# kscalelabs/kbot-joystick

Hardware: AMD Instinct MI355X
Metric: env-steps/sec (whole node), K-Bot joystick 8192 envs @1/2/4/8 MI355X (higher is better)
Workload: dtype f32; 1 GPU; kbot-headless, 8192 envs/GPU, flat ground, fixed joystick command (0.5,0,0), full iteration: 100-step rollout + PPO update (batch 512/GPU, 3 passes, LSTM hidden 256, depth 2); envs_per_gpu=8192, rollout_steps=100, batch_size_per_gpu=512, num_passes=3, hidden_size=256, deterministic_update=True, parallelism=env-sharded dp1, grad all-reduce per optimizer step

## Files before the change

kbot-joystick_amd/csrc/kbj_nn.hip:

```cpp
#include <hip/hip_runtime.h>
#include <vector>
#include <cmath>
#include <cstdlib>
#include <algorithm>
#include <type_traits>
#include "kbj_ctx.h"
#include "kbj_gemm.h"
#include "kbj_nn_kernels.h"
#include "kbj_lstm_seq.h"
#include "kbj_lstm_bwd16.h"
#include "kbj_deploy.h"
#include "kbj_terminal_value.h"

using namespace kbj;

namespace {

constexpr int MAXD = KBJ_MAX_DEPTH;

struct NetOff {
  size_t w_in, b_in, w_ih[MAXD], w_hh[MAXD], b[MAXD], w_out, b_out;
  int nin, nout, ld_obs;
};

// ... 443 lines not shown

int ev_record(kbj_ctx* ctx, hipEvent_t ev, hipStream_t on) { KBJ_HIP(ctx, hipEventRecord(ev, on)); return 0; }
int ev_wait(kbj_ctx* ctx, hipStream_t st, hipEvent_t ev) { KBJ_HIP(ctx, hipStreamWaitEvent(st, ev, 0)); return 0; }
int hop(kbj_ctx* ctx, hipStream_t from, hipStream_t to, hipEvent_t ev) { return ev_record(ctx, ev, from) || ev_wait(ctx, to, ev) ? -1 : 0; }

void pad_params(kbj_ctx* ctx, hipStream_t s, const float* user, float* internal) {
  NnWs& w = *ws_of(ctx);
  hipLaunchKernelGGL(pad_params_kernel, g1(w.nparams), dim3(256), 0, s, w.pad_desc, w.npad, const_cast<float*>(user), internal, w.nparams, 0);
}
void unpad_params(kbj_ctx* ctx, hipStream_t s, const float* internal, float* user) {
  NnWs& w = *ws_of(ctx);
  hipLaunchKernelGGL(pad_params_kernel, g1(w.nparams), dim3(256), 0, s, w.pad_desc, w.npad, user, const_cast<float*>(internal), w.nparams, 1);
}
void repitch_hc(kbj_ctx* ctx, hipStream_t s, const float* src, float* dst, int ws, int wd) {
  NnWs& w = *ws_of(ctx);
  const size_t rows = (size_t)2 * w.D * w.N;
  repitch_pad_launch(s, src, dst, rows, ws, wd);
}
kbj_carry pad_carry(kbj_ctx* ctx, hipStream_t s, const kbj_carry& c) {
  NnWs& w = *ws_of(ctx);
  kbj_carry p = c;
  for (int k = 0; k < 4; ++k)
    if (carry_hc(c, k) && w.phc[k]) { repitch_hc(ctx, s, carry_hc(c, k), w.phc[k], w.Hu, w.H); carry_hc(p, k) = w.phc[k]; }
  return p;
}
void unpad_carry(kbj_ctx* ctx, hipStream_t s, const kbj_carry& c) {
  NnWs& w = *ws_of(ctx);
  for (int k = 0; k < 4; ++k)
    if (carry_hc(c, k) && w.phc[k]) repitch_hc(ctx, s, w.phc[k], carry_hc(c, k), w.H, w.Hu);
}
kbj_traj pad_traj_carry0(kbj_ctx* ctx, hipStream_t s, const kbj_traj& tr) {
  NnWs& w = *ws_of(ctx);
  kbj_traj p = tr;
  for (int k = 0; k < 4; ++k)
    if (traj_carry0(tr, k) && w.pc0[k]) { repitch_hc(ctx, s, traj_carry0(tr, k), w.pc0[k], w.Hu, w.H); traj_carry0(p, k) = w.pc0[k]; }
  return p;
}


enum HeadKind {
  HEAD_SAMPLE,
  HEAD_VALUE,
  HEAD_LPF,
  HEAD_NONE
};
struct RolloutNet { hipStream_t lane; int type; bool step_kernel, folded0, mirrored, terminal; int tile; HeadKind head; float *hc, *lpf, *X, *G, *Out, *obs_m, **rH; };
struct RolloutPlan { RolloutNet net[4]; int nnets; bool serial; hipStream_t side; float* term_rows; hipEvent_t ev_term; };

RolloutPlan rollout_plan(kbj_ctx* ctx, const kbj_carry& carry, bool serial) {
  NnWs& w = *ws_of(ctx); const Sched& sc = w.sched;
  RolloutPlan p{};
  p.nnets = w.nnets; p.serial = serial;
  p.side = serial ? ctx->stream : ctx->side[0];
  p.term_rows = ctx->cfg_h.gae_terminal_value ? w.term_rows : nullptr;
  p.ev_term = p.term_rows && !serial ? ctx->ev_term : nullptr;
  const HeadKind heads[4] = {HEAD_SAMPLE, HEAD_VALUE, HEAD_LPF, HEAD_NONE};
  float* const lpf[4] = {carry.lpf_d, nullptr, carry.lpf_mirror_d, nullptr};
  for (int n = 0; n < p.nnets; ++n) {
    RolloutNet& q = p.net[n]; q.type = n & 1;
    q.lane = n == 0 ? ctx->stream : p.side;
    q.step_kernel = sc.rollout_step && n == 0;
    q.tile = sc.rollout_step && n > 0 ? 0 : -1;
    q.folded0 = q.step_kernel && sc.fold_actor && w.net[0].ld_obs == KBJ_LD_ACTOR;
    q.head = heads[n]; q.mirrored = n >= 2;
    q.terminal = n == 1 && p.term_rows != nullptr;
    q.hc = carry_hc(carry, n); q.lpf = lpf[n];
    q.X = w.rX[n]; q.G = w.rG[n]; q.Out = w.rOut[n]; q.obs_m = q.mirrored ? w.rObsM[q.type] : nullptr; q.rH = w.rH[n];
  }
  return p;
}

struct StepRows {
  const float *actor_obs, *critic_obs; float *aux, *action, *logp, *value, *actor_next, *critic_next, *aux_next, *qstate;
  uint32_t step_index; int argmax, parity;
  float* value_term;
};

void terminal_value_launch(hipStream_t st, const float* par, const NetOff& o, int N, int width, int D, const float* hc, const float* rows, const float* done_d, int done_stride,
                           float* value) {
  TermValueArgs a{};
  a.params = par; a.rows = rows; a.hc = hc; a.done = done_d; a.done_stride = done_stride; a.value = value;
  a.N = N; a.H = width; a.D = D; a.nin = o.nin; a.ld = o.ld_obs;
  a.w_in = o.w_in; a.b_in = o.b_in; a.w_out = o.w_out; a.b_out = o.b_out;
  for (int l = 0; l < D; ++l) { a.w_ih[l] = o.w_ih[l]; a.w_hh[l] = o.w_hh[l]; a.b[l] = o.b[l]; }
  critic_terminal_value_launch(st, a);
}

struct Rollout {
  kbj_ctx* ctx; const float* params; const RolloutPlan p; uint32_t seed;
  NnWs& w = *ws_of(ctx); const kbj_config& c = ctx->cfg_h; const int N = w.N, H = w.H;
  const HeadParams hp{c.min_std, c.max_std, c.var_scale, c.lpf_alpha, w.net[0].ld_obs};

  float* c_plane(const RolloutNet& q, int l) { return q.hc + (size_t)(2 * l + 1) * N * H; }
  float* h_plane(const RolloutNet& q, int l, bool partner) { return partner ? q.rH[l] : q.hc + (size_t)(2 * l) * N * H; }

  void fold_actor_weights(hipStream_t s) {
    if (!p.net[0].folded0) return;
    const NetOff& oa = w.net[0];
    GemmArgs g{params + oa.w_ih[0], params + oa.w_in, w.Weff, nullptr, 4 * H, oa.nin, H, H, oa.nin, oa.ld_obs, 0, 1, nullptr};
    gemm_launch<true, false>(s, g);
    matvec_launch(s, params + oa.w_ih[0], params + oa.b_in, params + oa.b[0], 4 * H, H, w.beff);
  }

  void repitch_input_weights(hipStream_t s, int k_lo = 0, int k_hi = 2) {
    for (int k = k_lo; k < k_hi; ++k) {
      const NetOff& o = w.net[k];
      if (o.nin != o.ld_obs) repitch_rows_launch(s, params + o.w_in, H, o.nin, o.ld_obs, w.WinP[k]);
    }
  }

  const float* observation_rows(const RolloutNet& q, const StepRows& v) {
    const float* obs = q.type == 0 ? v.actor_obs : v.critic_obs;
    if (!q.mirrored) return obs;
    mirror_rows_launch(q.lane, obs, q.obs_m, (size_t)N, w.net[q.type].ld_obs, w.mtab[q.type]);
    return q.obs_m;
  }

  void input_projection(const RolloutNet& q, const float* obs) {
    const NetOff& o = w.net[q.type];
    if (o.nin != o.ld_obs) linear_fwd(q.lane, obs, o.ld_obs, w.WinP[q.type], o.ld_obs, params + o.b_in, q.X, H, N, H, o.ld_obs, 0);
    else linear_fwd(q.lane, obs, o.ld_obs, params + o.w_in, o.nin, params + o.b_in, q.X, H, N, H, o.nin, 0);
  }

  const float* layers_step_kernel(const RolloutNet& q, const float* obs, int parity) {
    const NetOff& o = w.net[q.type];
    const float* x = q.X;
    for (int l = 0; l < w.D; ++l) {
      float* h_out = h_plane(q, l, parity == 0);
      StepArgs sa{x, H, 0, params + o.w_ih[l], H, params + o.w_hh[l], params + o.b[l], h_plane(q, l, parity != 0), h_out, c_plane(q, l), N};
      if (l == 0 && q.folded0) { sa.X = obs; sa.ldx = o.ld_obs; sa.kx = o.nin; sa.Wih = w.Weff; sa.ldw = o.ld_obs; sa.bias = w.beff; }
      if (lstm_step(ctx, q.lane, H, sa)) return nullptr;
      x = h_out;
    }
    return x;
  }

  const float* layers_gemm_cell(const RolloutNet& q) {
    const NetOff& o = w.net[q.type];
    const float* x = q.X;
    for (int l = 0; l < w.D; ++l) {
      float *h = h_plane(q, l, false), *cc = c_plane(q, l);
      GemmArgs g{x, params + o.w_ih[l], q.G, params + o.b[l], N, 4 * H, 2 * H, H, H, 4 * H, 0, 1, nullptr};
      g.A2 = h; g.B2 = params + o.w_hh[l]; g.k1 = H;
      g.x3 = w.sched.gemm_x3 ? 1 : 0;
      gemm_launch<true, true>(q.lane, g, q.tile);
      CellFwdArgs2 ca;
      ca.a[0] = CellFwdArgs{q.G, cc, h, cc, nullptr, nullptr, nullptr, nullptr, N, H};
      lstm_cell_fwd_launch(q.lane, ca, 1);
      x = h;
    }
    return x;
  }

  void head(const RolloutNet& q, const float* x, const float* obs, const StepRows& v) {
    const NetOff& o = w.net[q.type];
    if (q.head == HEAD_SAMPLE)
      actor_head_fused_launch(q.lane, x, H, params + o.w_out, params + o.b_out, obs, q.lpf, w.joint_bias_d, hp, seed, (uint32_t)c.env_id_offset, v.step_index, v.argmax, N,
                              v.action, v.logp);
    else if (q.head == HEAD_VALUE) critic_value_fused_launch(q.lane, x, H, params + o.w_out, params + o.b_out, N, v.value);
    else if (q.head == HEAD_LPF) {
      linear_fwd(q.lane, x, H, params + o.w_out, H, params + o.b_out, q.Out, 40, N, o.nout, H, 0);
      actor_head_lpf_launch(q.lane, q.Out, obs, q.lpf, w.joint_bias_d, c.lpf_alpha, N, w.net[0].ld_obs);
    }
  }

  int net_step(const RolloutNet& q, const StepRows& v) {
    const float* obs = observation_rows(q, v);
    if (!q.folded0) input_projection(q, obs);
    const float* x = q.step_kernel ? layers_step_kernel(q, obs, v.parity) : layers_gemm_cell(q);
    if (!x) return -1;
    head(q, x, obs, v);
    return 0;
  }

  void carry_reset(const RolloutNet& q, const float* done_d, int done_stride, int parity) {
    CarryPlanes cp;
    cp.n = 2 * w.D;
    for (int l = 0; l < w.D; ++l) { cp.p[2 * l] = h_plane(q, l, q.step_kernel && parity != 0); cp.p[2 * l + 1] = c_plane(q, l); }
    carry_reset_launch(q.lane, cp, N, H, q.lpf, done_d, done_stride);
  }

  int terminal_value(const RolloutNet& q, const StepRows& v) {
    if (!q.terminal) return 0;
    terminal_value_launch(q.lane, params, w.net[q.type], N, H, w.D, q.hc, p.term_rows, v.aux + KBJ_AUX_DONE, KBJ_AUX_SIZE, v.value_term);
    return p.ev_term ? ev_record(ctx, p.ev_term, q.lane) : 0;
  }
  int terminal_rows_free(hipStream_t s, bool first_step) { return p.ev_term && !first_step ? ev_wait(ctx, s, p.ev_term) : 0; }

  int planes_home() {
    for (int n = 0; n < p.nnets; ++n)
      for (int l = 0; l < w.D && p.net[n].step_kernel; ++l)
        KBJ_HIP(ctx, hipMemcpyAsync(h_plane(p.net[n], l, false), h_plane(p.net[n], l, true), (size_t)N * H * sizeof(float), hipMemcpyDeviceToDevice, ctx->stream));
    return 0;
  }

  int critic_tail(const float* critic_obs_d, const float* critic_hc_d, int hc_width, float* value_d) {
    RolloutNet q = p.net[1];
    q.hc = w.tail_hc;
    if (hc_width == H) KBJ_HIP(ctx, hipMemcpyAsync(w.tail_hc, critic_hc_d, (size_t)2 * w.D * N * H * sizeof(float), hipMemcpyDeviceToDevice, q.lane));
    else repitch_hc(ctx, q.lane, critic_hc_d, w.tail_hc, hc_width, H);
    StepRows v{};
    v.critic_obs = critic_obs_d; v.value = value_d;
    return net_step(q, v);
  }
};

int policy_step_body(kbj_ctx* ctx, const float* params_d, const float* actor_obs_d, const float* critic_obs_d, kbj_carry* carry, uint32_t seed,
                     uint32_t step_index, int argmax, float* action_d, float* logp_d, float* value_d) {
  kbj_nn_drop_prefetch(ctx);
  KbjTimed timed(ctx, true);
  Rollout r{ctx, params_d, rollout_plan(ctx, *carry, true), seed};
  r.repitch_input_weights(ctx->stream);
  r.fold_actor_weights(ctx->stream);
  const StepRows v{actor_obs_d, critic_obs_d, nullptr, action_d, logp_d, value_d, nullptr, nullptr, nullptr, nullptr, step_index, argmax, 0};
  for (int n = 0; n < r.p.nnets; ++n) if (r.net_step(r.p.net[n], v)) return -1;
  if (r.planes_home()) return -1;
  KBJ_CHECK_LAUNCH(ctx, "kbj_policy_step");
  return 0;
}

int rollout_body(kbj_ctx* ctx, const float* params_d, kbj_carry* carry, uint32_t seed, uint32_t first_step_index, kbj_traj* tr) {
  NnWs& w = *ws_of(ctx);
  const size_t N = w.N, T = tr->T, la = w.net[0].ld_obs, lc = w.net[1].ld_obs, lx = KBJ_AUX_SIZE;
  hipStream_t s = ctx->stream;
  kbj_nn_drop_prefetch(ctx);
  const struct { float* a; size_t ld; } rows[3] = {{tr->actor_obs_d, la}, {tr->critic_obs_d, lc}, {tr->aux_d, lx}};
  for (const auto& r : rows) KBJ_HIP(ctx, hipMemcpyAsync(r.a, r.a + T * N * r.ld, N * r.ld * sizeof(float), hipMemcpyDeviceToDevice, s));
  for (int n = 0; n < w.nnets; n += 2) {
    for (int k = n; k < n + 2; ++k)
      KBJ_HIP(ctx, hipMemcpyAsync(traj_carry0(*tr, k), carry_hc(*carry, k), 2 * w.D * N * w.H * sizeof(float), hipMemcpyDeviceToDevice, s));
    KBJ_HIP(ctx, hipMemcpyAsync(n ? tr->carry0_lpf_mirror_d : tr->carry0_lpf_d, n ? carry->lpf_mirror_d : carry->lpf_d, N * KBJ_NU * sizeof(float), hipMemcpyDeviceToDevice, s));
  }
  const char* pipe_env = getenv("KBJ_ROLLOUT_PIPELINE");
  Rollout r{ctx, params_d, rollout_plan(ctx, *carry, pipe_env && atoi(pipe_env) == 0), seed};
  const RolloutPlan& p = r.p;
  r.fold_actor_weights(s);
  r.repitch_input_weights(s);
  if (!p.serial && hop(ctx, s, p.side, ctx->ev_fork)) return -1;
  for (size_t t = 0; t < T; ++t) {
    const StepRows v{tr->actor_obs_d + t * N * la, tr->critic_obs_d + t * N * lc, tr->aux_d + t * N * lx, tr->action_d + t * N * KBJ_NU, tr->logp_d + t * N, tr->value_d + t * N,
                     tr->actor_obs_d + (t + 1) * N * la, tr->critic_obs_d + (t + 1) * N * lc, tr->aux_d + (t + 1) * N * lx,
                     tr->qstate_d ? tr->qstate_d + t * N * KBJ_QSTATE_SIZE : nullptr, first_step_index + (uint32_t)t, ctx->rollout_argmax, (int)(t & 1),
                     p.term_rows ? w.value_term + t * N : nullptr};
    const float* done = v.aux + KBJ_AUX_DONE;
    for (int n = 0; n < p.nnets; ++n) if (r.net_step(p.net[n], v)) return -1;
    if (r.terminal_rows_free(s, t == 0)) return -1;
    const int rc = kbj_env_step_all(ctx, s, v.action, v.aux, v.actor_next, v.critic_next, v.aux_next, v.qstate, p.term_rows);
    if (rc) return rc;
    r.carry_reset(p.net[0], done, KBJ_AUX_SIZE, (v.parity + 1) & 1);
    if (!p.serial && hop(ctx, s, p.side, ctx->ev_side[0])) return -1;
    for (int n = 1; n < p.nnets; ++n) {
      if (r.terminal_value(p.net[n], v)) return -1;
      r.carry_reset(p.net[n], done, KBJ_AUX_SIZE, (v.parity + 1) & 1);
    }
  }
  if (ctx->cfg_h.gae_tail_value && tr->value_tail_d && r.critic_tail(tr->critic_obs_d + T * N * lc, carry->critic_hc_d, w.H, tr->value_tail_d)) return -1;
  KBJ_CHECK_LAUNCH(ctx, "kbj_rollout");
  if (!p.serial && hop(ctx, p.side, s, ctx->ev_side[0])) return -1;
  if ((T & 1) && r.planes_home()) return -1;
  return kbj_rewards(ctx, tr->aux_d, (int)T, tr->reward_d, tr->reward_comps_d);
}

}

extern "C" {

int kbj_mirror_table(const void* model_blob, size_t model_bytes, int critic, int32_t* src_h, float* mul_h, float* add_h) {
  if (!model_blob || !src_h || !mul_h || !add_h || model_bytes != sizeof(kbj_model)) return kbj_fail(nullptr, "kbj_mirror_table: bad argument");
  std::vector<MirrorEntry> ta, tc;
  build_mirror_tables(*reinterpret_cast<const kbj_model*>(model_blob), ta, tc);
  const std::vector<MirrorEntry>& t = critic ? tc : ta;
  for (size_t k = 0; k < t.size(); ++k) { src_h[k] = t[k].src; mul_h[k] = t[k].mul; add_h[k] = t[k].add; }
  return (int)t.size();
}

size_t kbj_param_count(const kbj_config* cfg) { return layout_params(*cfg, cfg->hidden_size).nparams; }
size_t kbj_actor_param_count(const kbj_config* cfg) { return layout_params(*cfg, cfg->hidden_size).nactor; }

int kbj_init_params(kbj_ctx* ctx, uint32_t seed, float* params_d) {
  if (!ctx || !params_d) return kbj_fail(ctx, "kbj_init_params: null argument");
  KBJ_HIP(ctx, hipSetDevice(ctx->device));
  NnWs& w = *ws_of(ctx);
  const ParamLayout& u = w.user;
  int H = w.Hu;
  uint32_t leaf = 0;
  auto fill = [&](size_t off, size_t n, int fan_in) {
    init_uniform_launch(ctx->stream, params_d + off, n, 1.0f / std::sqrt((float)fan_in), seed, leaf++);
  };
  for (int n = 0; n < 2; ++n) {
    const NetOff& o = u.net[n];
    fill(o.w_in, (size_t)H * o.nin, o.nin); fill(o.b_in, H, o.nin);
    for (int l = 0; l < w.D; ++l) { fill(o.w_ih[l], (size_t)4 * H * H, H); fill(o.w_hh[l], (size_t)4 * H * H, H); fill(o.b[l], (size_t)4 * H, H); }
    fill(o.w_out, (size_t)o.nout * H, H); fill(o.b_out, o.nout, H);
  }
  KBJ_CHECK_LAUNCH(ctx, "init_uniform_kernel");
  return 0;
}

int kbj_policy_step(kbj_ctx* ctx, const float* params_d, const float* actor_obs_d, const float* critic_obs_d, kbj_carry* carry, uint32_t seed,
                    uint32_t step_index, int argmax, float* action_d, float* logp_d, float* value_d) {
  if (!ctx || !params_d || !actor_obs_d || !critic_obs_d || !carry || !action_d || !logp_d || !value_d) return kbj_fail(ctx, "kbj_policy_step: null argument");
  KBJ_HIP(ctx, hipSetDevice(ctx->device));
  NnWs& w = *ws_of(ctx);
  if (mirror_arrays_missing(w.mirror, carry, nullptr)) return kbj_fail(ctx, "kbj_policy_step: the mirror losses are enabled, the carry needs the mirror-branch arrays");
  if (!w.padded()) return policy_step_body(ctx, params_d, actor_obs_d, critic_obs_d, carry, seed, step_index, argmax, action_d, logp_d, value_d);
  pad_params(ctx, ctx->stream, params_d, w.pparams);
  kbj_carry pc = pad_carry(ctx, ctx->stream, *carry);
  const int rc = policy_step_body(ctx, w.pparams, actor_obs_d, critic_obs_d, &pc, seed, step_index, argmax, action_d, logp_d, value_d);
  unpad_carry(ctx, ctx->stream, *carry);
  return rc;
}

int kbj_carry_reset(kbj_ctx* ctx, kbj_carry* carry, const float* done_d, int done_stride) {
  if (!ctx || !carry || !done_d) return kbj_fail(ctx, "kbj_carry_reset: null argument");
  KBJ_HIP(ctx, hipSetDevice(ctx->device));
  NnWs& w = *ws_of(ctx);
  if (mirror_arrays_missing(w.mirror, carry, nullptr)) return kbj_fail(ctx, "kbj_carry_reset: the mirror losses are enabled, the carry needs the mirror-branch arrays");
  const kbj_carry pc = w.padded() ? pad_carry(ctx, ctx->stream, *carry) : *carry;
  Rollout r{ctx, nullptr, rollout_plan(ctx, pc, true), 0};
  for (int n = 0; n < r.p.nnets; ++n) r.carry_reset(r.p.net[n], done_d, done_stride, 0);
  if (w.padded()) unpad_carry(ctx, ctx->stream, *carry);
  KBJ_CHECK_LAUNCH(ctx, "carry_reset_kernel");
  return 0;
}

// ... 563 lines not shown
```

kbot-joystick_amd/csrc/kbj_nn_kernels.h:

```cpp
#pragma once
#include <hip/hip_runtime.h>
#include <stdint.h>
#include <cmath>
#include <vector>
#include "kbj_model.h"
#include "kbj_lstm_seq.h"

namespace kbj {

constexpr float kLog2Pi = 1.8378770664093453f;
inline dim3 g1(size_t n, int bs = 256) { return dim3((unsigned)((n + bs - 1) / bs)); }

__device__ __forceinline__ float sigmoidf_(float x) { return __builtin_amdgcn_rcpf(1.0f + __expf(-x)); }
__device__ __forceinline__ float tanhf_(float x) { float xc = fminf(fmaxf(x, -15.0f), 15.0f); return 1.0f - 2.0f * __builtin_amdgcn_rcpf(1.0f + __expf(2.0f * xc)); }
__device__ __forceinline__ float softplusf_(float x) { return x > 20.0f ? x : log1pf(expf(x)); }

__device__ __forceinline__ void lstm_cell_point(float pi, float pf, float pg, float po, float c_prev, float& i, float& f, float& gg, float& o, float& c, float& tc) {
  i = sigmoidf_(pi); f = sigmoidf_(pf); gg = tanhf_(pg); o = sigmoidf_(po);
  c = f * c_prev + i * gg;
  tc = tanhf_(c);
}
struct CellFwdArgs {
  float* G; const float* c_prev; float* h_out; float* c_out; float* hm_next; float* cm_next; float* tanhc; const float* keep;
  int M, H;
};
struct CellFwdArgs2 { CellFwdArgs a[2]; };
__global__ void lstm_cell_fwd_kernel(CellFwdArgs2 args) {
  const CellFwdArgs& a = args.a[blockIdx.y];
  int idx = blockIdx.x * blockDim.x + threadIdx.x;
  if (idx >= a.M * a.H) return;
  int m = idx / a.H, u = idx - m * a.H;
  float* g = a.G + (size_t)m * 4 * a.H;
  float i, f, gg, o, c, tc;
  lstm_cell_point(g[u], g[a.H + u], g[2 * a.H + u], g[3 * a.H + u], a.c_prev[idx], i, f, gg, o, c, tc);
  float h = o * tc;
  g[u] = i; g[a.H + u] = f; g[2 * a.H + u] = gg; g[3 * a.H + u] = o;
  a.h_out[idx] = h;
  a.c_out[idx] = c;
  if (a.hm_next) { float k = a.keep[m]; a.hm_next[idx] = h * k; a.cm_next[idx] = c * k; a.tanhc[idx] = tc; }
}
inline void lstm_cell_fwd_launch(hipStream_t st, const CellFwdArgs2& a, int count) {
  hipLaunchKernelGGL(lstm_cell_fwd_kernel, dim3((a.a[0].M * a.a[0].H + 255) / 256, count), dim3(256), 0, st, a);
}

__device__ __forceinline__ uint32_t nn_rotl32(uint32_t x, int r) { return (x << r) | (x >> (32 - r)); }
__device__ __forceinline__ void nn_threefry(uint32_t k0, uint32_t k1, uint32_t c0, uint32_t c1, uint32_t& o0, uint32_t& o1) {
  const int rot[8] = {13, 15, 26, 6, 17, 29, 16, 24};
  uint32_t ks[3] = {k0, k1, k0 ^ k1 ^ 0x1BD11BDAu};
  uint32_t x0 = c0 + ks[0], x1 = c1 + ks[1];
#pragma unroll
  for (int g = 0; g < 5; ++g) {
#pragma unroll
    for (int r = 0; r < 4; ++r) { x0 += x1; x1 = nn_rotl32(x1, rot[(g & 1) * 4 + r]); x1 ^= x0; }
    x0 += ks[(g + 1) % 3]; x1 += ks[(g + 2) % 3] + (uint32_t)(g + 1);
  }
  o0 = x0; o1 = x1;
}

struct HeadParams { float min_std, max_std, var_scale, alpha; int ld_obs; };
constexpr int HEAD_ENVS = 16;
constexpr int HEAD_WAVES = 4;
typedef float head_f32x4 __attribute__((ext_vector_type(4)));
__global__ __launch_bounds__(64 * HEAD_WAVES) void actor_head_fused_kernel(const float* __restrict__ hin , int H, const float* __restrict__ Wout ,
                                                                          const float* __restrict__ bout, const float* __restrict__ obs ,
                                                                          float* __restrict__ lpf, const float* __restrict__ joint_bias, HeadParams hp, uint32_t seed,
                                                                          uint32_t env_off, uint32_t step, int argmax, int N, float* __restrict__ action,
                                                                          float* __restrict__ logp) {
  __shared__ float outs[HEAD_WAVES][HEAD_ENVS][49];
  __shared__ float lps[HEAD_WAVES][HEAD_ENVS][KBJ_NU + 1];
  const int lane = threadIdx.x & 63, wv = threadIdx.x >> 6, g = lane >> 4, c = lane & 15;
  const int n0 = (blockIdx.x * HEAD_WAVES + wv) * HEAD_ENVS;
  if (n0 < N) {
    const float* arow = hin + (size_t)min(n0 + c, N - 1) * H + 4 * g;
    const float* brow[3] = {Wout + (size_t)c * H + 4 * g, Wout + (size_t)(16 + c) * H + 4 * g, Wout + (size_t)min(32 + c, 2 * KBJ_NU - 1) * H + 4 * g};
    head_f32x4 acc[3] = {{0, 0, 0, 0}, {0, 0, 0, 0}, {0, 0, 0, 0}};
    for (int k = 0; k < H; k += 16) {
      const head_f32x4 a = *reinterpret_cast<const head_f32x4*>(arow + k);
#pragma unroll
      for (int t = 0; t < 3; ++t) {
        const head_f32x4 b = *reinterpret_cast<const head_f32x4*>(brow[t] + k);
#pragma unroll
        for (int q = 0; q < 4; ++q) acc[t] = __builtin_amdgcn_mfma_f32_16x16x4f32(a[q], b[q], acc[t], 0, 0, 0);
      }
    }
#pragma unroll
    for (int t = 0; t < 3; ++t)
#pragma unroll
      for (int r = 0; r < 4; ++r) outs[wv][4 * g + r][16 * t + c] = acc[t][r];
  }
  __syncthreads();
  if (n0 < N) {
    for (int item = lane; item < HEAD_ENVS * KBJ_NU; item += 64) {
      const int e = item / KBJ_NU, j = item - e * KBJ_NU, n = n0 + e;
      float lp = 0;
      if (n < N) {
        const float om = outs[wv][e][j] + bout[j], os = outs[wv][e][KBJ_NU + j] + bout[KBJ_NU + j];
        float mean = om + joint_bias[j] + (j >= 10 ? obs[(size_t)n * hp.ld_obs + KBJ_OBS_CMD + 6 + (j - 10)] : 0.0f);
        float sd = fminf((softplusf_(os) + hp.min_std) * hp.var_scale, hp.max_std);
        float y0 = lpf[n * KBJ_NU + j];
        float y = y0 + hp.alpha * (mean - y0);
        lpf[n * KBJ_NU + j] = y;
        float a = y;
        if (!argmax) {
          uint32_t b0, b1;
          nn_threefry(seed ^ ((uint32_t)KBJ_RNG_ACTION * 0x9E3779B9u), env_off + (uint32_t)n, step, (uint32_t)j, b0, b1);
          float u1 = (float)((b0 >> 8) + 1u) * (1.0f / 16777216.0f), u2 = (float)(b1 >> 8) * (1.0f / 16777216.0f);
          a = y + sd * (sqrtf(-2.0f * logf(u1)) * cosf(6.283185307179586f * u2));
        }
        action[n * KBJ_NU + j] = a;
        float z = (a - y) / sd;
        lp = -0.5f * z * z - logf(sd) - 0.5f * kLog2Pi;
      }
      lps[wv][e][j] = lp;
    }
  }
  __syncthreads();
  if (n0 < N && lane < HEAD_ENVS && n0 + lane < N) {
    float lp = 0;
#pragma unroll
    for (int j = 0; j < KBJ_NU; ++j) lp += lps[wv][lane][j];
    logp[n0 + lane] = lp;
  }
}
inline int actor_head_fused_grid(int N) { return (N + HEAD_ENVS * HEAD_WAVES - 1) / (HEAD_ENVS * HEAD_WAVES); }
inline void actor_head_fused_launch(hipStream_t st, const float* hin, int H, const float* Wout, const float* bout, const float* obs, float* lpf, const float* joint_bias,
                                    HeadParams hp, uint32_t seed, uint32_t env_off, uint32_t step, int argmax, int N, float* action, float* logp) {
  hipLaunchKernelGGL(actor_head_fused_kernel, dim3(actor_head_fused_grid(N)), dim3(64 * HEAD_WAVES), 0, st, hin, H, Wout, bout, obs, lpf, joint_bias, hp, seed, env_off, step,
                     argmax, N, action, logp);
}

__global__ __launch_bounds__(256) void critic_value_fused_kernel(const float* __restrict__ hin , int H, const float* __restrict__ wout ,
                                                                 const float* __restrict__ bout, int N, float* __restrict__ value) {
  const int tid = blockIdx.x * blockDim.x + threadIdx.x, n = tid >> 5, j = tid & 31;
  float acc = 0;
  if (n < N)
    for (int c = j; c < H / 4; c += 32) {
      const float4 h = *reinterpret_cast<const float4*>(hin + (size_t)n * H + 4 * c), w = *reinterpret_cast<const float4*>(wout + 4 * c);
      acc = fmaf(h.x, w.x, acc); acc = fmaf(h.y, w.y, acc); acc = fmaf(h.z, w.z, acc); acc = fmaf(h.w, w.w, acc);
    }
  for (int o = 16; o > 0; o >>= 1) acc += __shfl_xor(acc, o);
  if (n < N && j == 0) value[n] = acc + bout[0];
}
inline void critic_value_fused_launch(hipStream_t st, const float* hin, int H, const float* wout, const float* bout, int N, float* value) {
  hipLaunchKernelGGL(critic_value_fused_kernel, dim3((unsigned)(((size_t)N * 32 + 255) / 256)), dim3(256), 0, st, hin, H, wout, bout, N, value);
}

__global__ void critic_value_kernel(const float* __restrict__ out, int ld, int N, float* __restrict__ value) {
  int n = blockIdx.x * blockDim.x + threadIdx.x;
  if (n < N) value[n] = out[(size_t)n * ld];
}
inline void critic_value_launch(hipStream_t st, const float* out, int ld, int N, float* value) {
  hipLaunchKernelGGL(critic_value_kernel, g1(N), dim3(256), 0, st, out, ld, N, value);
}

struct CarryPlanes { float* p[2 * KBJ_MAX_DEPTH]; int n; };
__global__ void carry_reset_kernel(CarryPlanes hc, int cnt, int H, float* __restrict__ lpf, const float* __restrict__ done, int stride) {
  const int row = blockIdx.x * (blockDim.x >> 6) + (threadIdx.x >> 6), lane = threadIdx.x & 63;
  if (row >= cnt || done[(size_t)row * stride] == 0.0f) return;
  for (int p = 0; p < hc.n; ++p)
    for (int k = lane; k < H; k += 64) hc.p[p][(size_t)row * H + k] = 0.0f;
  if (lpf && lane < KBJ_NU) lpf[(size_t)row * KBJ_NU + lane] = 0.0f;
}
inline void carry_reset_launch(hipStream_t st, const CarryPlanes& hc, int cnt, int H, float* lpf, const float* done, int stride) {
  hipLaunchKernelGGL(carry_reset_kernel, dim3((cnt + 3) / 4), dim3(256), 0, st, hc, cnt, H, lpf, done, stride);
}

__global__ void gather_rows_kernel(const float* __restrict__ src, const int* __restrict__ idx, int T, int N, int B, int w, int ld_src, int ld_dst, float* __restrict__ dst) {
  size_t i = (size_t)blockIdx.x * blockDim.x + threadIdx.x;
  size_t total = (size_t)T * B * w;
  if (i >= total) return;
  int k = i % w;
  size_t r = i / w;
  int b = r % B, t = r / B;
  dst[r * ld_dst + k] = src[((size_t)t * N + idx[b]) * ld_src + k];
}
__global__ void gather_rows4_kernel(const float4* __restrict__ src, const int* __restrict__ idx, int T, int N, int B, int w4, int ld_src4, int ld_dst4, float4* __restrict__ dst) {
  size_t i = (size_t)blockIdx.x * blockDim.x + threadIdx.x;
  size_t total = (size_t)T * B * w4;
  if (i >= total) return;
  int k = i % w4;
  size_t r = i / w4;
  int b = r % B, t = r / B;
  dst[r * ld_dst4 + k] = src[((size_t)t * N + idx[b]) * ld_src4 + k];
}
inline void gather_rows_launch(hipStream_t st, const float* src, const int* idx, int T, int N, int B, int wdt, int lds, float* dst, int ldd) {
  const size_t R = (size_t)T * B;
  if (wdt % 4 == 0 && lds % 4 == 0 && ldd % 4 == 0 && ((size_t)src & 15) == 0 && ((size_t)dst & 15) == 0)
    hipLaunchKernelGGL(gather_rows4_kernel, g1(R * (wdt / 4)), dim3(256), 0, st, reinterpret_cast<const float4*>(src), idx, T, N, B, wdt / 4, lds / 4, ldd / 4,
                       reinterpret_cast<float4*>(dst));
  else hipLaunchKernelGGL(gather_rows_kernel, g1(R * wdt), dim3(256), 0, st, src, idx, T, N, B, wdt, lds, ldd, dst);
}

struct GatherSmallArgs {
  const float *action, *logp, *value, *adv, *target, *aux;
  float *action_o, *logp_o, *value_o, *adv_o, *target_o, *keep_o;
};
__global__ void gather_small_kernel(GatherSmallArgs a, const int* __restrict__ idx, int T, int N, int B, int c0, int c1) {
  const int W = c1 - c0;
  size_t i = (size_t)blockIdx.x * blockDim.x + threadIdx.x;
  if (i >= (size_t)T * B * W) return;
  size_t r = i / W;
  int c = c0 + (int)(i - r * W), b = (int)(r % B);
  size_t src = (r / B) * N + idx[b];
  if (c < KBJ_NU) a.action_o[r * KBJ_NU + c] = a.action[src * KBJ_NU + c];
  else if (c == KBJ_NU) { if (a.logp) a.logp_o[r] = a.logp[src]; }
  else if (c == KBJ_NU + 1) { if (a.value) a.value_o[r] = a.value[src]; }
  else if (c == KBJ_NU + 2) { if (a.adv) a.adv_o[r] = a.adv[src]; }
  else if (c == KBJ_NU + 3) { if (a.target) a.target_o[r] = a.target[src]; }
  else a.keep_o[r] = a.aux[src * KBJ_AUX_SIZE + KBJ_AUX_DONE] != 0 ? 0.0f : 1.0f;
}
inline void gather_small_launch(hipStream_t st, const GatherSmallArgs& a, const int* idx, int T, int N, int B, int c0, int c1) {
  hipLaunchKernelGGL(gather_small_kernel, g1((size_t)T * B * (c1 - c0)), dim3(256), 0, st, a, idx, T, N, B, c0, c1);
}
struct GatherCarryArgs { const float* src[8 * KBJ_MAX_DEPTH + 2]; float* dst[8 * KBJ_MAX_DEPTH + 2]; int nplanes, nlpf; };
__global__ void gather_carry_kernel(GatherCarryArgs a, const int* __restrict__ idx, int B, int H) {
  int p = blockIdx.y;
  int w = p < a.nplanes ? H : KBJ_NU;
  int i = blockIdx.x * blockDim.x + threadIdx.x;
  if (i >= B * w) return;
  int b = i / w, k = i - b * w;
  a.dst[p][i] = a.src[p][(size_t)idx[b] * w + k];
}
inline void gather_carry_launch(hipStream_t st, const GatherCarryArgs& a, const int* idx, int B, int H) {
  hipLaunchKernelGGL(gather_carry_kernel, dim3((B * H + 255) / 256, a.nplanes + a.nlpf), dim3(256), 0, st, a, idx, B, H);
}

__global__ void actor_head_pre_kernel(const float* __restrict__ out, const float* __restrict__ obs, const float* __restrict__ joint_bias, HeadParams hp,
                                      int R, float* __restrict__ y, float* __restrict__ sd) {
  size_t i = (size_t)blockIdx.x * blockDim.x + threadIdx.x;
  if (i >= (size_t)R * KBJ_NU) return;
  size_t r = i / KBJ_NU;
  int j = (int)(i - r * KBJ_NU);
  y[i] = out[r * 40 + j] + joint_bias[j] + (j >= 10 ? obs[r * hp.ld_obs + KBJ_OBS_CMD + 6 + (j - 10)] : 0.0f);
  sd[i] = fminf((softplusf_(out[r * 40 + KBJ_NU + j]) + hp.min_std) * hp.var_scale, hp.max_std);
}
inline void actor_head_pre_launch(hipStream_t st, const float* out, const float* obs, const float* joint_bias, HeadParams hp, int R, float* y, float* sd) {
  hipLaunchKernelGGL(actor_head_pre_kernel, g1((size_t)R * KBJ_NU), dim3(256), 0, st, out, obs, joint_bias, hp, R, y, sd);
}
__global__ void actor_head_train_fwd_kernel(const float* __restrict__ keep, const float* __restrict__ lpf0, HeadParams hp, int T, int B, float* __restrict__ y) {
  int i = blockIdx.x * blockDim.x + threadIdx.x;
  if (i >= B * KBJ_NU) return;
  int b = i / KBJ_NU, j = i % KBJ_NU;
  float state = lpf0[i];
  constexpr int U = 10;
  for (int t0 = 0; t0 < T; t0 += U) {
    float mean[U], kp[U];
#pragma unroll
    for (int u = 0; u < U; ++u) {
      int t = t0 + u;
      if (t < T) { size_t r = (size_t)t * B + b; mean[u] = y[r * KBJ_NU + j]; kp[u] = keep[r]; }
    }
#pragma unroll
    for (int u = 0; u < U; ++u) {
      int t = t0 + u;
      if (t < T) {
        float yy = state + hp.alpha * (mean[u] - state);
        y[((size_t)t * B + b) * KBJ_NU + j] = yy;
        state = yy * kp[u];
      }
    }
  }
}
inline void actor_head_train_fwd_launch(hipStream_t st, const float* keep, const float* lpf0, HeadParams hp, int T, int B, float* y) {
  hipLaunchKernelGGL(actor_head_train_fwd_kernel, g1((size_t)B * KBJ_NU, 64), dim3(64), 0, st, keep, lpf0, hp, T, B, y);
}
__global__ void gaussian_logp_kernel(const float* __restrict__ y, const float* __restrict__ sd, const float* __restrict__ act, int R,
                                     float* __restrict__ logp, float* __restrict__ ent) {
  int r = blockIdx.x * blockDim.x + threadIdx.x;
  if (r >= R) return;
  float lp = 0, en = 0;
  for (int j = 0; j < KBJ_NU; ++j) {
    float s = sd[(size_t)r * KBJ_NU + j], z = (act[(size_t)r * KBJ_NU + j] - y[(size_t)r * KBJ_NU + j]) / s;
    lp += -0.5f * z * z - logf(s) - 0.5f * kLog2Pi;
    en += 0.5f + 0.5f * kLog2Pi + logf(s);
  }
  logp[r] = lp; ent[r] = en;
}
inline void gaussian_logp_launch(hipStream_t st, const float* y, const float* sd, const float* act, int R, float* logp, float* ent) {
  hipLaunchKernelGGL(gaussian_logp_kernel, g1(R), dim3(256), 0, st, y, sd, act, R, logp, ent);
}

// ... 535 lines not shown
```

Before: 2.333 million env-steps/s.

## Restructure actor head kernel: one env tile per block, split MFMA across waves, overlap RNG

The fused actor head kernel now handles one 16-env tile per block. Three waves each compute one 16-column slice of the output projection, and the fourth wave precomputes the Gaussian noise, which the MFMA waves also help with. The kernel is templated on hidden size so loads are unrolled and prefetched a block ahead, and the per-item inputs are loaded before the GEMM. The aim is to hide load latency and move the threefry/Box-Muller work off the serial epilogue, at the cost of more blocks, more registers and a launch failure path for unsupported hidden sizes.

```diff
diff --git a/kbot-joystick_amd/csrc/kbj_nn.hip b/kbot-joystick_amd/csrc/kbj_nn.hip
--- a/kbot-joystick_amd/csrc/kbj_nn.hip
+++ b/kbot-joystick_amd/csrc/kbj_nn.hip
@@ -619,16 +619,18 @@
     return x;
   }
 
-  void head(const RolloutNet& q, const float* x, const float* obs, const StepRows& v) {
+  int head(const RolloutNet& q, const float* x, const float* obs, const StepRows& v) {
     const NetOff& o = w.net[q.type];
-    if (q.head == HEAD_SAMPLE)
-      actor_head_fused_launch(q.lane, x, H, params + o.w_out, params + o.b_out, obs, q.lpf, w.joint_bias_d, hp, seed, (uint32_t)c.env_id_offset, v.step_index, v.argmax, N,
-                              v.action, v.logp);
-    else if (q.head == HEAD_VALUE) critic_value_fused_launch(q.lane, x, H, params + o.w_out, params + o.b_out, N, v.value);
+    if (q.head == HEAD_SAMPLE) {
+      if (!actor_head_fused_launch(q.lane, x, H, params + o.w_out, params + o.b_out, obs, q.lpf, w.joint_bias_d, hp, seed, (uint32_t)c.env_id_offset, v.step_index, v.argmax, N,
+                                   v.action, v.logp))
+        return kbj_fail(ctx, "actor head: the kernel is built for hidden_size 64, 128, ..., 512");
+    } else if (q.head == HEAD_VALUE) critic_value_fused_launch(q.lane, x, H, params + o.w_out, params + o.b_out, N, v.value);
     else if (q.head == HEAD_LPF) {
       linear_fwd(q.lane, x, H, params + o.w_out, H, params + o.b_out, q.Out, 40, N, o.nout, H, 0);
       actor_head_lpf_launch(q.lane, q.Out, obs, q.lpf, w.joint_bias_d, c.lpf_alpha, N, w.net[0].ld_obs);
     }
+    return 0;
   }
 
   int net_step(const RolloutNet& q, const StepRows& v) {
@@ -636,8 +638,7 @@
     if (!q.folded0) input_projection(q, obs);
     const float* x = q.step_kernel ? layers_step_kernel(q, obs, v.parity) : layers_gemm_cell(q);
     if (!x) return -1;
-    head(q, x, obs, v);
-    return 0;
+    return head(q, x, obs, v);
   }
 
   void carry_reset(const RolloutNet& q, const float* done_d, int done_stride, int parity) {
diff --git a/kbot-joystick_amd/csrc/kbj_nn_kernels.h b/kbot-joystick_amd/csrc/kbj_nn_kernels.h
--- a/kbot-joystick_amd/csrc/kbj_nn_kernels.h
+++ b/kbot-joystick_amd/csrc/kbj_nn_kernels.h
@@ -60,73 +60,109 @@
 struct HeadParams { float min_std, max_std, var_scale, alpha; int ld_obs; };
 constexpr int HEAD_ENVS = 16;
 constexpr int HEAD_WAVES = 4;
+constexpr int HEAD_KB = 64;
+constexpr int HEAD_ITEMS = HEAD_ENVS * KBJ_NU;
 typedef float head_f32x4 __attribute__((ext_vector_type(4)));
-__global__ __launch_bounds__(64 * HEAD_WAVES) void actor_head_fused_kernel(const float* __restrict__ hin , int H, const float* __restrict__ Wout ,
-                                                                          const float* __restrict__ bout, const float* __restrict__ obs ,
-                                                                          float* __restrict__ lpf, const float* __restrict__ joint_bias, HeadParams hp, uint32_t seed,
-                                                                          uint32_t env_off, uint32_t step, int argmax, int N, float* __restrict__ action,
-                                                                          float* __restrict__ logp) {
-  __shared__ float outs[HEAD_WAVES][HEAD_ENVS][49];
-  __shared__ float lps[HEAD_WAVES][HEAD_ENVS][KBJ_NU + 1];
-  const int lane = threadIdx.x & 63, wv = threadIdx.x >> 6, g = lane >> 4, c = lane & 15;
-  const int n0 = (blockIdx.x * HEAD_WAVES + wv) * HEAD_ENVS;
-  if (n0 < N) {
+__device__ __forceinline__ float head_deviate(uint32_t seed, uint32_t env, uint32_t step, uint32_t j) {
+  uint32_t b0, b1;
+  nn_threefry(seed ^ ((uint32_t)KBJ_RNG_ACTION * 0x9E3779B9u), env, step, j, b0, b1);
+  float u1 = (float)((b0 >> 8) + 1u) * (1.0f / 16777216.0f), u2 = (float)(b1 >> 8) * (1.0f / 16777216.0f);
+  return sqrtf(-2.0f * logf(u1)) * cosf(6.283185307179586f * u2);
+}
+template <int H>
+__global__ __launch_bounds__(64 * HEAD_WAVES, 4) void actor_head_fused_kernel(const float* __restrict__ hin , const float* __restrict__ Wout ,
+                                                                             const float* __restrict__ bout, const float* __restrict__ obs ,
+                                                                             float* __restrict__ lpf, const float* __restrict__ joint_bias, HeadParams hp, uint32_t seed,
+                                                                             uint32_t env_off, uint32_t step, int argmax, int N, float* __restrict__ action,
+                                                                             float* __restrict__ logp) {
+  static_assert(H % HEAD_KB == 0, "whole fetch blocks");
+  constexpr int NB = H / HEAD_KB, NF = HEAD_KB / 16;
+  constexpr int AHEAD = NB <= 4 ? 2 : 1;
+  __shared__ float outs[HEAD_ENVS][49];
+  __shared__ float devs[HEAD_ITEMS];
+  __shared__ float lps[HEAD_ENVS][KBJ_NU + 1];
+  const int tid = threadIdx.x, lane = tid & 63, wv = __builtin_amdgcn_readfirstlane(tid >> 6), g = lane >> 4, c = lane & 15;
+  const int n0 = blockIdx.x * HEAD_ENVS;
+  const bool two = wv == 0;
+  float y0[2], cmd[2], bm[2], bs[2], jb[2];
+#pragma unroll
+  for (int p = 0; p < 2; ++p)
+    if (p == 0 || two) {
+      const int item = tid + 256 * p, e = item / KBJ_NU, j = item - e * KBJ_NU, n = min(n0 + e, N - 1);
+      y0[p] = lpf[n * KBJ_NU + j];
+      cmd[p] = obs[(size_t)n * hp.ld_obs + KBJ_OBS_CMD + 6 + (j >= 10 ? j - 10 : 0)];
+      bm[p] = bout[j]; bs[p] = bout[KBJ_NU + j]; jb[p] = joint_bias[j];
+    }
+  if (wv < 3) {
     const float* arow = hin + (size_t)min(n0 + c, N - 1) * H + 4 * g;
-    const float* brow[3] = {Wout + (size_t)c * H + 4 * g, Wout + (size_t)(16 + c) * H + 4 * g, Wout + (size_t)min(32 + c, 2 * KBJ_NU - 1) * H + 4 * g};
-    head_f32x4 acc[3] = {{0, 0, 0, 0}, {0, 0, 0, 0}, {0, 0, 0, 0}};
-    for (int k = 0; k < H; k += 16) {
-      const head_f32x4 a = *reinterpret_cast<const head_f32x4*>(arow + k);
-#pragma unroll
-      for (int t = 0; t < 3; ++t) {
-        const head_f32x4 b = *reinterpret_cast<const head_f32x4*>(brow[t] + k);
-#pragma unroll
-        for (int q = 0; q < 4; ++q) acc[t] = __builtin_amdgcn_mfma_f32_16x16x4f32(a[q], b[q], acc[t], 0, 0, 0);
+    const float* brow = Wout + (size_t)min(16 * wv + c, 2 * KBJ_NU - 1) * H + 4 * g;
+    head_f32x4 a[NB][NF], b[NB][NF];
+#pragma unroll
+    for (int blk = 0; blk < (NB < AHEAD ? NB : AHEAD); ++blk)
+#pragma unroll
+      for (int f = 0; f < NF; ++f) {
+        a[blk][f] = *reinterpret_cast<const head_f32x4*>(arow + blk * HEAD_KB + 16 * f);
+        b[blk][f] = *reinterpret_cast<const head_f32x4*>(brow + blk * HEAD_KB + 16 * f);
       }
-    }
-#pragma unroll
-    for (int t = 0; t < 3; ++t)
-#pragma unroll
-      for (int r = 0; r < 4; ++r) outs[wv][4 * g + r][16 * t + c] = acc[t][r];
+    if (!argmax) { const int item = 64 * wv + lane, e = item / KBJ_NU; devs[item] = head_deviate(seed, env_off + (uint32_t)(n0 + e), step, (uint32_t)(item - e * KBJ_NU)); }
+    head_f32x4 acc = {0, 0, 0, 0};
+#pragma unroll
+    for (int blk = 0; blk < NB; ++blk) {
+      if (blk + AHEAD < NB) {
+#pragma unroll
+        for (int f = 0; f < NF; ++f) {
+          a[blk + AHEAD][f] = *reinterpret_cast<const head_f32x4*>(arow + (blk + AHEAD) * HEAD_KB + 16 * f);
+          b[blk + AHEAD][f] = *reinterpret_cast<const head_f32x4*>(brow + (blk + AHEAD) * HEAD_KB + 16 * f);
+        }
+        __builtin_amdgcn_sched_barrier(0);
+      }
+#pragma unroll
+      for (int f = 0; f < NF; ++f)
+#pragma unroll
+        for (int q = 0; q < 4; ++q) acc = __builtin_amdgcn_mfma_f32_16x16x4f32(a[blk][f][q], b[blk][f][q], acc, 0, 0, 0);
+    }
+#pragma unroll
+    for (int r = 0; r < 4; ++r) outs[4 * g + r][16 * wv + c] = acc[r];
+  } else if (!argmax) {
+#pragma unroll
+    for (int p = 0; p < 2; ++p) { const int item = 192 + 64 * p + lane, e = item / KBJ_NU; devs[item] = head_deviate(seed, env_off + (uint32_t)(n0 + e), step, (uint32_t)(item - e * KBJ_NU)); }
   }
   __syncthreads();
-  if (n0 < N) {
-    for (int item = lane; item < HEAD_ENVS * KBJ_NU; item += 64) {
-      const int e = item / KBJ_NU, j = item - e * KBJ_NU, n = n0 + e;
+#pragma unroll
+  for (int p = 0; p < 2; ++p)
+    if (p == 0 || two) {
+      const int item = tid + 256 * p, e = item / KBJ_NU, j = item - e * KBJ_NU, n = n0 + e;
       float lp = 0;
       if (n < N) {
-        const float om = outs[wv][e][j] + bout[j], os = outs[wv][e][KBJ_NU + j] + bout[KBJ_NU + j];
-        float mean = om + joint_bias[j] + (j >= 10 ? obs[(size_t)n * hp.ld_obs + KBJ_OBS_CMD + 6 + (j - 10)] : 0.0f);
+        const float om = outs[e][j] + bm[p], os = outs[e][KBJ_NU + j] + bs[p];
+        float mean = om + jb[p] + (j >= 10 ? cmd[p] : 0.0f);
         float sd = fminf((softplusf_(os) + hp.min_std) * hp.var_scale, hp.max_std);
-        float y0 = lpf[n * KBJ_NU + j];
-        float y = y0 + hp.alpha * (mean - y0);
+        float y = y0[p] + hp.alpha * (mean - y0[p]);
         lpf[n * KBJ_NU + j] = y;
         float a = y;
-        if (!argmax) {
-          uint32_t b0, b1;
-          nn_threefry(seed ^ ((uint32_t)KBJ_RNG_ACTION * 0x9E3779B9u), env_off + (uint32_t)n, step, (uint32_t)j, b0, b1);
-          float u1 = (float)((b0 >> 8) + 1u) * (1.0f / 16777216.0f), u2 = (float)(b1 >> 8) * (1.0f / 16777216.0f);
-          a = y + sd * (sqrtf(-2.0f * logf(u1)) * cosf(6.283185307179586f * u2));
-        }
+        if (!argmax) a = y + sd * devs[item];
         action[n * KBJ_NU + j] = a;
         float z = (a - y) / sd;
         lp = -0.5f * z * z - logf(sd) - 0.5f * kLog2Pi;
       }
-      lps[wv][e][j] = lp;
-    }
-  }
+      lps[e][j] = lp;
+    }
   __syncthreads();
-  if (n0 < N && lane < HEAD_ENVS && n0 + lane < N) {
+  if (tid < HEAD_ENVS && n0 + tid < N) {
     float lp = 0;
 #pragma unroll
-    for (int j = 0; j < KBJ_NU; ++j) lp += lps[wv][lane][j];
-    logp[n0 + lane] = lp;
-  }
-}
-inline int actor_head_fused_grid(int N) { return (N + HEAD_ENVS * HEAD_WAVES - 1) / (HEAD_ENVS * HEAD_WAVES); }
-inline void actor_head_fused_launch(hipStream_t st, const float* hin, int H, const float* Wout, const float* bout, const float* obs, float* lpf, const float* joint_bias,
+    for (int j = 0; j < KBJ_NU; ++j) lp += lps[tid][j];
+    logp[n0 + tid] = lp;
+  }
+}
+inline int actor_head_fused_grid(int N) { return (N + HEAD_ENVS - 1) / HEAD_ENVS; }
+inline bool actor_head_fused_launch(hipStream_t st, const float* hin, int H, const float* Wout, const float* bout, const float* obs, float* lpf, const float* joint_bias,
                                     HeadParams hp, uint32_t seed, uint32_t env_off, uint32_t step, int argmax, int N, float* action, float* logp) {
-  hipLaunchKernelGGL(actor_head_fused_kernel, dim3(actor_head_fused_grid(N)), dim3(64 * HEAD_WAVES), 0, st, hin, H, Wout, bout, obs, lpf, joint_bias, hp, seed, env_off, step,
-                     argmax, N, action, logp);
+  const dim3 grid(actor_head_fused_grid(N)), block(64 * HEAD_WAVES);
+  return dispatch_hidden(H, [&](auto hc) {
+    hipLaunchKernelGGL((actor_head_fused_kernel<decltype(hc)::value>), grid, block, 0, st, hin, Wout, bout, obs, lpf, joint_bias, hp, seed, env_off, step, argmax, N, action, logp);
+    return true;
+  });
 }
 
 __global__ __launch_bounds__(256) void critic_value_fused_kernel(const float* __restrict__ hin , int H, const float* __restrict__ wout ,
```

Measured after the change: 2.340 million env-steps/s, median of 6. No clear change (+0.3%).
